# JonasGeiping/breaching

Hardware: NVIDIA B200
Metric: reconstruction iters/sec (ResNet-18 224x224, invertinggradients) (higher is better)
Workload: dtype tf32

## Files before the change

breaching_b200/csrc/engine.cu:

```cuda
#include <math.h>
#include <stdlib.h>
#include <string.h>

#include <limits>
#include <string>
#include <vector>

#include "../../include/breaching_b200.h"
#include "common.cuh"
#include "igemm.cuh"
#include "layers.cuh"
#include "tokens.cuh"
#include "objective.cuh"
#include "augment.cuh"

namespace bre {
void set_pdl(bool on);
static thread_local std::string g_last_error;
void set_error(const std::string& msg) { g_last_error = msg; }
static int g_pdl = -1;
bool use_pdl() {
  if (g_pdl < 0) {
    const char* e = getenv("BRE_PDL");
    g_pdl = e ? (atoi(e) != 0) : 1;
// ... 51 lines not shown
struct bre_engine {
  int device = 0;
  cudaStream_t stream = nullptr;
  std::vector<TensorBuf> t;
  std::vector<bre_op_desc> ops;
  std::vector<ParamInfo> params;
  std::vector<BnBuf> bn;
  std::vector<int*> pool_idx;
  int logits = -1;
  bre_attack_cfg cfg;
  std::vector<void*> allocs;

  long long P_pad = 0, max_param = 0, max_tensor = 0;
  float *W = nullptr, *g = nullptr, *G = nullptr, *V = nullptr, *stage = nullptr, *chunk_w = nullptr;
  float *Wt = nullptr, *Vt = nullptr;
  std::vector<float*> ms_Wt;
  bool tc_round_env = [] { const char* e = getenv("BRE_TC_ROUND"); return e ? atoi(e) != 0 : true; }();
  bool tc_round() const { return gemm_backend == 1 && tc_round_env; }
  float *p = nullptr, *loss_n = nullptr;
  long long* labels = nullptr;
  int seq_len = 0;
  std::vector<float*> tok_a, tok_b;
  float* soft_q = nullptr;
  float* soft_q_buf = nullptr;
  float* label_grad = nullptr;
  int n_labels = 0;
  int logits_valid = 0;
  int classes() const { return logits_valid > 0 ? logits_valid : td(logits).C; }
  bool joint = false;
  float *ell = nullptr, *ell_m = nullptr, *ell_v = nullptr, *ell_best = nullptr;
  long long n_ell = 0;
  long long nx = 0;
  int xN = 0, xC = 0, xH = 0, xW = 0;
  float *x = nullptr, *gradx = nullptr, *gradx_task = nullptr, *m = nullptr, *v = nullptr, *best = nullptr;
  float *history = nullptr, *lr_table = nullptr, *lo = nullptr, *hi = nullptr;
  int n_lr = 0, lr_cap = 0;
  Scalars* sc = nullptr;
  float* ws = nullptr;
  int ws_tiles = 0;
  int* gemm_counters = nullptr;
  float* red_partials = nullptr;
  int* red_counters = nullptr;
  double* dpartials = nullptr;
  int* dcounter = nullptr;
  DiLayer* di_layers_dev = nullptr;
  int n_di = 0;
  float* feat_measured = nullptr;
  long long feat_numel = 0;
  int feat_op = -1;
  cudaStream_t side = nullptr;
  std::vector<cudaEvent_t> ev_fork;
  cudaEvent_t ev_join = nullptr;
  bool overlap_wgrad = true;
  bool fuse_bnact = [] { const char* e = getenv("BRE_FUSE_BNACT"); return e ? atoi(e) != 0 : false; }();
  float* ws2 = nullptr;
  int* gemm_counters2 = nullptr;
  float* red_partials2 = nullptr;
  int* red_counters2 = nullptr;
  struct StepBufs {
    std::vector<float*> val, d;
    std::vector<int*> idx;
    std::vector<float*> bn_scale, bn_shift;
    float* p = nullptr; float* loss_n = nullptr; long long* labels = nullptr;
  };
  int ms_steps = 0;
  float ms_lr = 0.f;
  std::vector<float*> ms_W;
  std::vector<StepBufs> ms_bufs;
  std::vector<long long> ms_offset;
  float* ms_D = nullptr;
  float* gradx_step = nullptr;
  float* W0 = nullptr;
  struct BnPrep { int gamma_off, beta_off, C; const float* inv; const float* nrm; float* scale; float* shift; };
  std::vector<BnPrep*> ms_bnprep_dev;
  int n_bn_layers = 0;
  bool want_tangent_G = false;
  int stem_op = -1, stem_Kp = 0;
  float *xcol = nullptr, *dcol = nullptr, *Wcol = nullptr, *Vcol = nullptr, *Gcol = nullptr;
  bool stem_cols_env = [] { const char* e = getenv("BRE_STEM_COLS"); return e ? atoi(e) != 0 : true; }();
  bool use_stem_cols(size_t i) { return gemm_backend == 1 && stem_cols_env && (int)i == stem_op && !is_precise(i); }
  GemmArgs stem_geom(const bre_op_desc& op) const {
    GemmArgs a;
    memset(&a, 0, sizeof(a));
    const bre_tensor_desc& to = td(op.tout);
    a.g = ConvGeom{to.N, to.H, to.W, stem_Kp, to.H, to.W, to.C, 1, 1, 1, 0};
    a.x_sN = (long long)to.H * to.W * stem_Kp; a.x_sP = stem_Kp; a.x_sC = 1;
    a.nsrc = 1;
    a.ws = ws; a.counters = gemm_counters; a.ws_tiles = ws_tiles; a.splits = 0;
    return a;
  }
  int stem_unfold(const bre_op_desc& op) {
    const bre_tensor_desc &ti = td(op.tin), &to = td(op.tout);
    BRE_LAUNCH(launch_stem_im2col(t[0].val, xcol, ti.N, ti.C, ti.H, ti.W, to.H, to.W, op.R, op.S, op.stride, op.pad, stem_Kp, tc_round(), stream));
    return 0;
  }
  int stem_pad(const float* src, float* dst, const bre_op_desc& op, cudaStream_t st) {
    BRE_LAUNCH(launch_stem_pad_rows(src, dst, td(op.tout).C, op.R * op.S * td(op.tin).C, stem_Kp, false, tc_round(), st));
    return 0;
  }
  int stem_fold(const bre_op_desc& op, float* grad_out) {
    const bre_tensor_desc &ti = td(op.tin), &to = td(op.tout);
    BRE_LAUNCH(launch_stem_col2im(dcol, grad_out, ti.N, ti.C, ti.H, ti.W, to.H, to.W, op.R, op.S, op.stride, op.pad, stem_Kp, stream));
    return 0;
  }
  int precise_first = [] { const char* e = getenv("BRE_PRECISE_FIRST"); return e ? atoi(e) : 0; }();
  int precise_last = [] { const char* e = getenv("BRE_PRECISE_LAST"); return e ? atoi(e) : 0; }();
  mutable std::vector<char> precise_op;
// ... 116 lines not shown
    }
    if (stem_op >= 0 && stem_cols_env && !is_precise((size_t)stem_op)) rnd_d[ops[stem_op].tout] = 1;
  }
  bool round_val(int tensor) { if (rnd_val.size() != t.size()) compute_round_flags(); return tc_round() && rnd_val[tensor]; }
  bool round_d(int tensor) { if (rnd_d.size() != t.size()) compute_round_flags(); return tc_round() && rnd_d[tensor]; }

  GemmArgs conv_geom(const bre_op_desc& op) const {
    GemmArgs a;
    memset(&a, 0, sizeof(a));
    const bre_tensor_desc &ti = td(op.tin), &to = td(op.tout);
    ConvGeom& g = a.g;
    if (op.kind == BRE_OP_LINEAR) {
      g.N = ti.N; g.H = 1; g.W = 1; g.Ci = ti.C * ti.H * ti.W; g.Ho = 1; g.Wo = 1; g.Co = to.C;
      g.R = 1; g.S = 1; g.stride = 1; g.pad = 0;
      a.x_sN = g.Ci; a.x_sP = g.Ci; a.x_sC = 1;
    } else {
      g.N = ti.N; g.H = ti.H; g.W = ti.W; g.Ci = ti.C; g.Ho = to.H; g.Wo = to.W; g.Co = to.C;
      g.R = op.R; g.S = op.S; g.stride = op.stride; g.pad = op.pad;
      if (op.tin == 0) { a.x_sN = (long long)ti.C * ti.H * ti.W; a.x_sP = 1; a.x_sC = ti.H * ti.W; }
      else { a.x_sN = (long long)ti.H * ti.W * ti.C; a.x_sP = ti.C; a.x_sC = 1; }
    }
    a.nsrc = 1;
    a.ws = ws; a.counters = gemm_counters; a.ws_tiles = ws_tiles; a.splits = 0;
    a.force_fp32 = is_precise(op_index(op)) ? 1 : 0;
    return a;
  }
  int gemm(const GemmArgs& a) { return gemm_on(a, stream); }
  bool weight_prefetch = [] { const char* e = getenv("BRE_TC_WPREFETCH"); return e ? atoi(e) != 0 : true; }();
  bool v_settled = false;
  bool inside(const float* p, const float* base, long long n) const { return base != nullptr && p >= base && p < base + n; }
  unsigned static_weights(const GemmArgs& a) const {
    if (!weight_prefetch || ms_steps > 0 || a.mode == GEMM_WGRAD) return 0u;
    unsigned mask = 0;
    for (int s = 0; s < a.nsrc; ++s) {
      const float* p = a.wgt[s];
      const bool model = inside(p, W, P_pad) || inside(p, Wt, P_pad) || (Wcol != nullptr && p == Wcol);
      const bool direction = v_settled && (inside(p, V, P_pad) || inside(p, Vt, P_pad));
      if (model || direction) mask |= 1u << s;
    }
    return mask;
  }
  int gemm_on(const GemmArgs& a, cudaStream_t st) {
    if (linear_tall_supported(a)) return launch_linear_tall(a, st);
    if (linear_small_preferred(a)) return launch_linear_small(a, st);
    if (gemm_backend == 1 && !a.force_fp32 && igemm_tc_supported(a)) {
      GemmArgs b = a;
      b.wgt_static = static_weights(a);
      return launch_igemm_tc(b, st);
    }
    return launch_igemm_simt(a, st);
  }

  bool fuses_with_next(size_t i, const GemmArgs& a) const {
    if (!fuse_bnact || gemm_backend != 1 || i + 1 >= ops.size()) return false;
    const bre_op_desc& nx = ops[i + 1];
    return nx.kind == BRE_OP_BNACT && nx.tin == ops[i].tout && !nx.bn_train && igemm_tc_supported(a);
  }
  int consumers_of(int tensor) const {
    int n = 0;
    for (const bre_op_desc& o : ops) n += (o.tin == tensor) + (o.res == tensor);
    return n;
  }

  BnTrainArgs bn_train_args(const bre_op_desc& op) {
    const bre_tensor_desc& to = td(op.tout);
    const BnBuf& b = bn[op.bn_buffer];
    BnTrainArgs a;
    memset(&a, 0, sizeof(a));
    a.P = (long long)to.N * to.H * to.W; a.C = to.C; a.relu = op.relu != 0;
    a.in = t[op.tin].val; a.out = t[op.tout].val;
    a.inv = b.inv; a.nrm = b.nrm; a.scale = b.scale;
    a.v_gamma = Vp(op.gamma); a.v_beta = Vp(op.beta);
    a.sum_du = Gp(op.beta); a.sum_duxh = Gp(op.gamma);
    a.m1 = b.di_cm; a.m2 = b.di_cv; a.b1 = b.tb1; a.b2 = b.tb2;
    a.dout = t[op.tout].d; a.tdout = t[op.tout].td; a.xd = t[op.tin].tval;
    return a;
  }

  BnConsts bn_consts(const bre_op_desc& op) const {
    BnConsts c{nullptr, nullptr, nullptr, nullptr};
    if (op.has_bn) { const BnBuf& b = bn[op.bn_buffer]; c = BnConsts{b.scale, b.shift, b.inv, b.nrm}; }
    return c;
  }
  PoolGeom pool_geom(const bre_op_desc& op) const {
    const bre_tensor_desc &ti = td(op.tin), &to = td(op.tout);
    return PoolGeom{ti.N, ti.H, ti.W, ti.C, to.H, to.W, op.R, op.stride, op.pad};
  }
  bool need_task_grad() const { return cfg.task_regularization != 0.f; }
  float value_task_reg() const { return cfg.objective_excludes_task ? 0.f : cfg.task_regularization; }

  int sweep_forward() {
    for (size_t i = 0; i < ops.size(); ++i) {
      const bre_op_desc& op = ops[i];
      const bre_tensor_desc& to = td(op.tout);
      const long long Pout = (long long)to.N * to.H * to.W;
      switch (op.kind) {
        case BRE_OP_CONV:
        case BRE_OP_LINEAR: {
          GemmArgs a = conv_geom(op);
          a.mode = GEMM_FPROP;
          a.act[0] = t[op.tin].val; a.wgt[0] = Wg(op);
          if (use_stem_cols(i)) {
            BRE_TRY(stem_unfold(op));
            if (ms_steps > 0) BRE_TRY(stem_pad(Wp(op.w), Wcol, op, stream));
            a = stem_geom(op);
            a.mode = GEMM_FPROP;
            a.act[0] = xcol; a.wgt[0] = Wcol;
          }
          a.bias = op.b >= 0 ? Wp(op.b) : nullptr;
// ... 1390 lines not shown
```

breaching_b200/csrc/igemm.cuh:

```cuda
#pragma once
#include "common.cuh"

namespace bre {

enum GemmMode { GEMM_FPROP = 0, GEMM_DGRAD = 1, GEMM_WGRAD = 2 };

struct ConvGeom {
  int N, H, W, Ci;
  int Ho, Wo, Co;
  int R, S, stride, pad;
};

struct GemmEpilogue {
  int kind;
  int has_bn, relu;
  int round_out;
  float* out2;
  const float* res;
  const float* scale;
  const float* shift;
  const float* inv;
  const float* nrm;
  const float* v_gamma;
  const float* v_beta;
  const float* pre;
  const float* post;
};

struct GemmArgs {
  int mode;
  GemmEpilogue epi;
  ConvGeom g;
  int nsrc;
  const float* act[2];
  const float* wgt[2];
  long long x_sN;
  int x_sP, x_sC;
  float* out;
  const float* bias;
  int accumulate;
  float* ws;
  int* counters;
  int ws_tiles;
  int splits;
  int force_fp32;
  unsigned wgt_static;
};

constexpr int IG_BM = 64, IG_BN = 64, IG_BK = 16, IG_THREADS = 256;

int launch_igemm_simt(const GemmArgs& a, cudaStream_t stream);
bool linear_small_supported(const GemmArgs& a);
int launch_linear_small(const GemmArgs& a, cudaStream_t stream);
bool linear_small_preferred(const GemmArgs& a);
bool linear_tall_supported(const GemmArgs& a);
int launch_linear_tall(const GemmArgs& a, cudaStream_t stream);
int launch_igemm_tc(const GemmArgs& a, cudaStream_t stream);
bool igemm_tc_supported(const GemmArgs& a);

inline void gemm_dims(const GemmArgs& a, int& M, int& Nc, int& K) {
  const ConvGeom& g = a.g;
  if (a.mode == GEMM_FPROP) { M = g.N * g.Ho * g.Wo; Nc = g.Co; K = g.R * g.S * g.Ci; }
  else if (a.mode == GEMM_DGRAD) { M = g.N * g.H * g.W; Nc = g.Ci; K = g.R * g.S * g.Co; }
  else { M = g.Co; Nc = g.R * g.S * g.Ci; K = g.N * g.Ho * g.Wo; }
}

}
```

breaching_b200/csrc/igemm_tc.cu:

```cuda
#include <stdlib.h>
#include <string.h>

#include <array>
#include <map>
#include <mutex>
#include <type_traits>

#include <cuda.h>

#include "igemm.cuh"

namespace bre {

namespace {

constexpr int TC_BM = 128;
constexpr int TC_BK = 32;
constexpr int TC_STAGES = 4;
constexpr int TC_MAX_STAGES = 8;
constexpr int TC_THREADS = 128;
constexpr int TC_BLOCK = TC_THREADS + 32;

struct TcDims {
  int M, Nc, K;
// ... 106 lines not shown
constexpr int TC_MAXCLS = 4;
struct ClsPlan {
  int ncls, stride;
  int tile0[TC_MAXCLS + 1];
  int Hc[TC_MAXCLS], Wc[TC_MAXCLS], y0[TC_MAXCLS], x0[TC_MAXCLS];
  int Ty[TC_MAXCLS], Tx[TC_MAXCLS], Ly[TC_MAXCLS], Lx[TC_MAXCLS], ey[TC_MAXCLS], ex[TC_MAXCLS];
};
struct TcMapsCls {
  CUtensorMap act[2 * TC_MAXCLS];
  CUtensorMap wgt[2];
};

__device__ __forceinline__ void mbar_expect_tx(uint64_t* bar, uint32_t bytes) {
  asm volatile("mbarrier.arrive.expect_tx.shared::cta.b64 _, [%0], %1;" ::"r"(smem_u32(bar)), "r"(bytes) : "memory");
}
__device__ __forceinline__ void tma_im2col(uint32_t dst, const CUtensorMap* tm, uint64_t* bar, int c, int w, int h, int n, int ow, int oh) {
  asm volatile(
      "cp.async.bulk.tensor.4d.shared::cluster.global.im2col.mbarrier::complete_tx::bytes [%0], [%1, {%3, %4, %5, %6}], [%2], {%7, %8};"
      ::"r"(dst), "l"(reinterpret_cast<uint64_t>(tm)), "r"(smem_u32(bar)), "r"(c), "r"(w), "r"(h), "r"(n), "h"((uint16_t)ow), "h"((uint16_t)oh)
      : "memory");
}
__device__ __forceinline__ void tma_tile2d(uint32_t dst, const CUtensorMap* tm, uint64_t* bar, int c0, int c1) {
  asm volatile("cp.async.bulk.tensor.2d.shared::cluster.global.tile.mbarrier::complete_tx::bytes [%0], [%1, {%3, %4}], [%2];"
               ::"r"(dst), "l"(reinterpret_cast<uint64_t>(tm)), "r"(smem_u32(bar)), "r"(c0), "r"(c1) : "memory");
}
__device__ __forceinline__ void tma_tile3d(uint32_t dst, const CUtensorMap* tm, uint64_t* bar, int c0, int c1, int c2) {
  asm volatile("cp.async.bulk.tensor.3d.shared::cluster.global.tile.mbarrier::complete_tx::bytes [%0], [%1, {%3, %4, %5}], [%2];"
               ::"r"(dst), "l"(reinterpret_cast<uint64_t>(tm)), "r"(smem_u32(bar)), "r"(c0), "r"(c1), "r"(c2) : "memory");
}

template <int NV>
__device__ __forceinline__ void fused_bnact(const GemmEpilogue& e, long long row, int n, float (&v)[NV]) {
  const long long o = row + n;
#pragma unroll
  for (int j = 0; j < NV; ++j) {
    float u = v[j];
    if (e.kind == 1) {
      if (e.has_bn) u = fmaf(u, __ldg(e.scale + n + j), __ldg(e.shift + n + j));
      if (e.res != nullptr) u += e.res[o + j];
      u = e.relu ? fmaxf(u, 0.f) : u;
      v[j] = e.round_out ? tf32_rna(u) : u;
    } else {
      if (e.has_bn) {
        const float xhat = fmaf(e.pre[o + j], __ldg(e.inv + n + j), __ldg(e.nrm + n + j));
        u = fmaf(__ldg(e.scale + n + j), u, fmaf(__ldg(e.v_gamma + n + j), xhat, __ldg(e.v_beta + n + j)));
      }
      if (e.res != nullptr) u += e.res[o + j];
      if (e.relu && !(e.post[o + j] > 0.f)) u = 0.f;
      v[j] = e.round_out ? tf32_rna(u) : u;
    }
  }
}

#ifdef BRE_TC_TRACE
__device__ long long g_tc_trace[16];
#define TC_MARK(i, cond) do { if ((cond) && blockIdx.x == 0 && blockIdx.y == 0 && blockIdx.z == 0) g_tc_trace[i] = clock64(); } while (0)
#else
#define TC_MARK(i, cond) do { } while (0)
#endif

template <int MODE, int BN, bool TMA, bool CLS = false>
__global__ void __launch_bounds__(TC_BLOCK) igemm_tc_kernel(GemmArgs a, TcDims d, int proxy_fence,
                                                            const __grid_constant__ std::conditional_t<CLS, TcMapsCls, TcMaps> maps, ClsPlan plan) {
  static_assert(!CLS || (MODE == GEMM_DGRAD && TMA), "per-class gathers: strided dgrad with the TMA producer only");
  constexpr uint32_t A_BYTES = TC_BM * TC_BK * 4, B_BYTES = BN * TC_BK * 4;
  extern __shared__ __align__(1024) uint8_t smem[];
  uint8_t* sA = smem;
  const int nst = 1 << d.stage_shift, stage_mask = nst - 1;
  uint8_t* sB = smem + nst * A_BYTES;
  __shared__ __align__(8) uint64_t bar_full[TC_MAX_STAGES];
  __shared__ __align__(8) uint64_t bar_empty[TC_MAX_STAGES];
  __shared__ __align__(8) uint64_t bar_done;
  __shared__ uint32_t s_tmem;

  TC_MARK(0, threadIdx.x == 0);
  pdl_launch_dependents();
  const ConvGeom g = a.g;
  const int tid = threadIdx.x, warp = tid >> 5;
  const int n0 = blockIdx.y * BN, z = blockIdx.z;
  int m0 = blockIdx.x * TC_BM;
  int kb_begin = z * d.kblocks_per_split;
  int kb_end = min(d.total_kblocks, kb_begin + d.kblocks_per_split);
  const int HoWo = g.Ho * g.Wo, HW = g.H * g.W;
  int cls = 0, cHc = 0, cWc = 0, cTy = 0, cTx = 0, cls_kps = 0, Mrows = d.M;
  if (CLS) {
#pragma unroll
    for (int c = 1; c < TC_MAXCLS; ++c)
      if (c < plan.ncls && (int)blockIdx.x >= plan.tile0[c]) cls = c;
    m0 = ((int)blockIdx.x - plan.tile0[cls]) * TC_BM;
    cHc = plan.Hc[cls]; cWc = plan.Wc[cls]; cTy = plan.Ty[cls]; cTx = plan.Tx[cls];
    Mrows = g.N * cHc * cWc;
    cls_kps = cTy * cTx * (g.Co / TC_BK);
    const int total = cls_kps * a.nsrc, per = (total + (int)gridDim.z - 1) / (int)gridDim.z;
    kb_begin = z * per;
    kb_end = min(total, kb_begin + per);
  }

  if (tid == 0) {
#pragma unroll
    for (int s = 0; s < TC_MAX_STAGES; ++s) { mbar_init(&bar_full[s], TMA ? 1 : TC_THREADS); mbar_init(&bar_empty[s], 1); }
    mbar_init(&bar_done, 1);
    fence_barrier_init();
  }
  if (warp == 0) tmem_alloc(&s_tmem, BN);
  tc_fence_before();
  __syncthreads();
  tc_fence_after();
  const uint32_t tmem_d = s_tmem;
  TC_MARK(1, threadIdx.x == 0);

  constexpr uint32_t a_mn = (MODE == GEMM_WGRAD) ? 1u : 0u;
  constexpr uint32_t b_mn = (MODE == GEMM_FPROP) ? 0u : 1u;
  constexpr uint32_t idesc = (1u << 4) | (2u << 7) | (2u << 10) | (a_mn << 15) | (b_mn << 16) | ((uint32_t)(BN >> 3) << 17) |
                             ((uint32_t)(TC_BM >> 4) << 24);

  constexpr int A_VEC = TC_BM * TC_BK / 4 / TC_THREADS;
  constexpr int B_VEC = BN * TC_BK / 4 / TC_THREADS;
// ... 122 lines not shown
    } else if (MODE == GEMM_DGRAD) {
#pragma unroll
      for (int h = 0; h < BN / 32; ++h) tma_tile3d(pb + h * 4096, &maps.wgt[st.src], bar, n0 + 32 * h, st.rs, st.c0);
    } else {
      const uint32_t pa = smem_u32(sA) + stage * A_BYTES;
#pragma unroll
      for (int h = 0; h < TC_BM / 32; ++h) tma_tile2d(pa + h * 4096, &maps.wgt[st.src], bar, m0 + 32 * h, st.c0);
    }
  };
  auto issue_act_tma = [&](int stage, const KbState& st) {
    uint64_t* bar = &bar_full[stage];
    const uint32_t pa = smem_u32(sA) + stage * A_BYTES, pb = smem_u32(sB) + stage * B_BYTES;
    if (MODE == GEMM_FPROP) {
      tma_im2col(pa, &maps.act[st.src], bar, st.c0, base_w, base_h, base_n, st.s, st.r);
    } else if (MODE == GEMM_DGRAD) {
      if (CLS) tma_im2col(pa, &maps.act[2 * cls + st.src], bar, st.c0, base_w, base_h, base_n, cTx - 1 - st.s, cTy - 1 - st.r);
      else tma_im2col(pa, &maps.act[st.src], bar, st.c0, base_w, base_h, base_n, g.S - 1 - st.s, g.R - 1 - st.r);
    } else {
#pragma unroll
      for (int h = 0; h < BN / 32; ++h)
        tma_im2col(pb + h * 4096, &maps.act[st.src], bar, wg_c[h], st.q * g.stride - g.pad, st.p * g.stride - g.pad, st.img, wg_s[h], wg_r[h]);
    }
  };

  if (TMA && tid == 0 && (proxy_fence & 2)) {
    for (int sidx = 0; sidx < a.nsrc; ++sidx) {
      asm volatile("prefetch.tensormap [%0];" ::"l"(reinterpret_cast<uint64_t>(&maps.act[(CLS ? 2 * cls : 0) + sidx])) : "memory");
      asm volatile("prefetch.tensormap [%0];" ::"l"(reinterpret_cast<uint64_t>(&maps.wgt[sidx])) : "memory");
    }
  }
  const int nprod = (proxy_fence >> 2) & 7;
  const bool producer = TMA && (tid & 31) == 0 && warp < nprod && warp < nkb;
  KbState pst;
  memset(&pst, 0, sizeof(pst));
  uint32_t pre_wgt = 0;
  if (producer) {
    pst = kb_init(kb_begin + warp);
    if (MODE != GEMM_WGRAD && a.wgt_static != 0) {
      KbState st = pst;
      for (int i = warp; i < nkb && i < nst; i += nprod) {
        if ((a.wgt_static >> st.src) & 1) {
          mbar_expect_tx(&bar_full[i], A_BYTES + B_BYTES);
          issue_wgt_tma(i, st);
          pre_wgt |= 1u << i;
        }
        for (int u = 0; u < nprod; ++u) kb_advance(st);
      }
    }
  }

  pdl_wait();
  TC_MARK(2, threadIdx.x == 0);

  auto issue_block = [&](int stage) {
    const int src = it_src;
    const int kch = (MODE == GEMM_DGRAD) ? g.Co : g.Ci;
    const int kbase = (MODE == GEMM_WGRAD) ? it_c0 : it_rs * kch + it_c0;
    const float* __restrict__ act = a.act[src];
    const float* __restrict__ wgt = a.wgt[src];
    const uint32_t pa = smem_u32(sA + stage * A_BYTES), pb = smem_u32(sB + stage * B_BYTES);
    if (MODE == GEMM_FPROP) {
      const int r = it_rs / g.S, s = it_rs - r * g.S;
      const int tapoff = (r * g.W + s) * a.x_sP + it_c0;
#pragma unroll
      for (int j = 0; j < A_VEC; ++j) {
        const bool ok = (a_taps[j] >> it_rs) & 1ull;
        cp_async16(pa + off_k128(grow + 16 * j, gcol), ok ? act + (a_off[j] + tapoff) : act, ok ? 16u : 0u);
      }
      const float* q = wgt + (long long)(n0 + grow) * d.K + kbase + gcol * 4;
#pragma unroll
      for (int j = 0; j < B_VEC; ++j) cp_async16(pb + off_k128(grow + 16 * j, gcol), q + (long long)(16 * j) * d.K, 16u);
    } else if (MODE == GEMM_DGRAD) {
      const int rs = it_rs, k0 = it_c0;
      const int r = rs / g.S, s = rs - r * g.S;
      if (g.stride == 1) {
        const int tapoff = k0 - (r * g.Wo + s) * g.Co;
#pragma unroll
        for (int j = 0; j < A_VEC; ++j) {
          const bool ok = (a_taps[j] >> rs) & 1ull;
          cp_async16(pa + off_k128(grow + 16 * j, gcol), ok ? act + (a_off[j] + tapoff) : act, ok ? 16u : 0u);
        }
      } else {
        const bool st2 = g.stride == 2;
#pragma unroll
        for (int j = 0; j < A_VEC; ++j) {
          const bool ok = (a_taps[j] >> rs) & 1ull;
          const int dr = r - (a_yx[j] >> 16), ds = s - (a_yx[j] & 0xffff);
          const int tr = st2 ? dr >> 1 : dr / g.stride, ts = st2 ? ds >> 1 : ds / g.stride;
          cp_async16(pa + off_k128(grow + 16 * j, gcol), ok ? act + (a_off[j] + k0 - (tr * g.Wo + ts) * g.Co) : act, ok ? 16u : 0u);
        }
      }
      const int n4 = tid & 15, kk = tid >> 4;
#pragma unroll
      for (int j = 0; j < B_VEC; ++j) {
        const int k = kk + 8 * j;
        const float* gb = wgt + ((long long)(k0 + k) * (g.R * g.S) + rs) * g.Ci + n0 + n4 * 4;
        cp_async16(pb + off_mnmajor<BN>(4 * n4, k), gb, 16u);
      }
    } else {
      {
        const int m4 = tid & 31, kk = tid >> 5;
#pragma unroll
        for (int j = 0; j < A_VEC; ++j) {
          const int k = kk + 4 * j;
          const int pix = kbase + k;
          const bool kok = pix < d.K;
// ... 78 lines not shown
        const int stage = i & stage_mask;
        if (i >= nst) mbar_wait(&bar_empty[stage], (uint32_t)(((i >> d.stage_shift) - 1) & 1));
        issue_block(stage);
        cp_async_arrive(&bar_full[stage]);
      }
    }
    mbar_wait(&bar_done, 0);
    TC_MARK(6, tid == 0);
    tc_fence_after();
  }

  const int splits = gridDim.z;
  const int tile = blockIdx.y * gridDim.x + blockIdx.x;
  const uint32_t lane_base = tmem_d + ((uint32_t)(warp * 32) << 16);
  float v[32];
  const int m = m0 + tid;
  const bool row_ok = m < Mrows;
  const bool is_loader = warp < TC_THREADS / 32;
  auto out_row = [&](int mm, long long& row, int& cs) {
    if (CLS) {
      const int per = cHc * cWc;
      const int img = mm / per, rem = mm - img * per;
      const int iy = rem / cWc, ix = rem - iy * cWc;
      row = img * a.x_sN + (long long)((plan.y0[cls] + plan.stride * iy) * g.W + plan.x0[cls] + plan.stride * ix) * a.x_sP;
      cs = a.x_sC;
    } else if (MODE == GEMM_DGRAD) {
      const int img = mm / HW;
      row = img * a.x_sN + (long long)(mm - img * HW) * a.x_sP;
      cs = a.x_sC;
    } else {
      row = (long long)mm * d.Nc;
      cs = 1;
    }
  };
  if (!is_loader) {
  } else if (splits == 1) {
    long long row = 0;
    int cs = 1;
    if (row_ok) out_row(m, row, cs);
#pragma unroll
    for (int c = 0; c < BN; c += 32) {
      if (nkb > 0) tmem_ld32(lane_base + c, v);
      else {
#pragma unroll
        for (int j = 0; j < 32; ++j) v[j] = 0.f;
      }
      if (!row_ok) continue;
      const int n = n0 + c;
      if (MODE == GEMM_FPROP && a.bias != nullptr) {
#pragma unroll
        for (int j = 0; j < 32; ++j) v[j] += __ldg(a.bias + n + j);
      }
      float* op = a.out + row + (long long)n * cs;
      if (MODE == GEMM_FPROP && a.epi.kind != 0) {
        if (a.out != nullptr) {
#pragma unroll
          for (int j = 0; j < 32; j += 4) *reinterpret_cast<float4*>(op + j) = make_float4(v[j], v[j + 1], v[j + 2], v[j + 3]);
        }
        fused_bnact<32>(a.epi, row, n, v);
        float* op2 = a.epi.out2 + row + n;
#pragma unroll
        for (int j = 0; j < 32; j += 4) *reinterpret_cast<float4*>(op2 + j) = make_float4(v[j], v[j + 1], v[j + 2], v[j + 3]);
      } else if (cs == 1) {
#pragma unroll
        for (int j = 0; j < 32; j += 4) {
          float4 t = make_float4(v[j], v[j + 1], v[j + 2], v[j + 3]);
          if (a.accumulate) {
            const float4 o = *reinterpret_cast<const float4*>(op + j);
            t.x += o.x; t.y += o.y; t.z += o.z; t.w += o.w;
          }
          *reinterpret_cast<float4*>(op + j) = t;
        }
      } else {
#pragma unroll
        for (int j = 0; j < 32; ++j) {
          float* q = op + (long long)j * cs;
          *q = a.accumulate ? *q + v[j] : v[j];
        }
      }
    }
  } else {
    float* part = reinterpret_cast<float*>(sA);
#pragma unroll
    for (int c = 0; c < BN; c += 32) {
      if (nkb > 0) tmem_ld32(lane_base + c, v);
      else {
#pragma unroll
        for (int j = 0; j < 32; ++j) v[j] = 0.f;
      }
#pragma unroll
      for (int j = 0; j < 32; j += 4) {
        const int chunk = ((c + j) >> 2) ^ (tid & (BN / 4 - 1) & 15);
        *reinterpret_cast<float4*>(part + tid * BN + chunk * 4) = make_float4(v[j], v[j + 1], v[j + 2], v[j + 3]);
      }
    }
  }
  if (splits > 1) {
    TC_MARK(7, tid == 0);
    cluster_sync_all();
    TC_MARK(8, tid == 0);
    if (is_loader) {
      auto reduce_rows = [&](auto s_tag) {
        constexpr int S = decltype(s_tag)::value;
        constexpr int C4 = BN / 4, SLOTS = (TC_BM / S) * C4 / TC_THREADS > 0 ? (TC_BM / S) * C4 / TC_THREADS : 1;
        static_assert(BN >= 64 || S <= 8, "narrow tiles: at most 8 splits");
        const uint32_t part_s = smem_u32(sA);
        float4 t[SLOTS][S];
        int rr[SLOTS], cc[SLOTS];
#pragma unroll
        for (int sl = 0; sl < SLOTS; ++sl) {
          const int slot = tid + sl * TC_THREADS;
          rr[sl] = z * (TC_BM / S) + slot / C4;
          cc[sl] = slot % C4;
          const uint32_t local = part_s + (uint32_t)(rr[sl] * BN + ((cc[sl] ^ (rr[sl] & (BN / 4 - 1) & 15)) << 2)) * 4u;
#pragma unroll
          for (int q = 0; q < S; ++q) t[sl][q] = ld_dsmem4(local, (uint32_t)q);
        }
#pragma unroll
        for (int sl = 0; sl < SLOTS; ++sl) {
          const int r = rr[sl], c4 = cc[sl];
          if (m0 + r >= Mrows) continue;
          float4 acc4 = t[sl][0];
#pragma unroll
          for (int q = 1; q < S; ++q) { acc4.x += t[sl][q].x; acc4.y += t[sl][q].y; acc4.z += t[sl][q].z; acc4.w += t[sl][q].w; }
          const int n = n0 + c4 * 4;
          if (MODE == GEMM_FPROP && a.bias != nullptr) {
            acc4.x += __ldg(a.bias + n); acc4.y += __ldg(a.bias + n + 1); acc4.z += __ldg(a.bias + n + 2); acc4.w += __ldg(a.bias + n + 3);
          }
          long long row;
          int cs;
          out_row(m0 + r, row, cs);
          float* op = a.out + row + (long long)n * cs;
          if (MODE == GEMM_FPROP && a.epi.kind != 0) {
            if (a.out != nullptr) *reinterpret_cast<float4*>(op) = acc4;
            float vv[4] = {acc4.x, acc4.y, acc4.z, acc4.w};
            fused_bnact<4>(a.epi, row, n, vv);
            *reinterpret_cast<float4*>(a.epi.out2 + row + n) = make_float4(vv[0], vv[1], vv[2], vv[3]);
          } else if (cs == 1) {
            if (a.accumulate) {
              const float4 o = *reinterpret_cast<const float4*>(op);
              acc4.x += o.x; acc4.y += o.y; acc4.z += o.z; acc4.w += o.w;
            }
            *reinterpret_cast<float4*>(op) = acc4;
          } else {
            const float vv[4] = {acc4.x, acc4.y, acc4.z, acc4.w};
#pragma unroll
            for (int j = 0; j < 4; ++j) {
              float* qq = op + (long long)j * cs;
              *qq = a.accumulate ? *qq + vv[j] : vv[j];
            }
          }
        }
      };
      switch (splits) {
        case 2: reduce_rows(std::integral_constant<int, 2>{}); break;
        case 4: reduce_rows(std::integral_constant<int, 4>{}); break;
        case 8: reduce_rows(std::integral_constant<int, 8>{}); break;
        default:
          if constexpr (BN >= 64) reduce_rows(std::integral_constant<int, 16>{});
          break;
      }
    }
    TC_MARK(9, tid == 0);
    cluster_sync_all();
  }
  tc_fence_before();
  __syncthreads();
  if (warp == 0) tmem_dealloc(tmem_d, BN);
  TC_MARK(10, tid == 0);
}

inline bool aligned16(const void* p) { return (reinterpret_cast<uintptr_t>(p) & 15) == 0; }

typedef CUresult (*EncodeIm2colFn)(CUtensorMap*, CUtensorMapDataType, cuuint32_t, void*, const cuuint64_t*, const cuuint64_t*, const int*,
                                   const int*, cuuint32_t, cuuint32_t, const cuuint32_t*, CUtensorMapInterleave, CUtensorMapSwizzle,
                                   CUtensorMapL2promotion, CUtensorMapFloatOOBfill);
typedef CUresult (*EncodeTiledFn)(CUtensorMap*, CUtensorMapDataType, cuuint32_t, void*, const cuuint64_t*, const cuuint64_t*,
                                  const cuuint32_t*, const cuuint32_t*, CUtensorMapInterleave, CUtensorMapSwizzle,
                                  CUtensorMapL2promotion, CUtensorMapFloatOOBfill);

struct TmaApi {
  EncodeIm2colFn im2col = nullptr;
  EncodeTiledFn tiled = nullptr;
  int driver = 0;
  bool ok = false;
};
const TmaApi& tma_api() {
  static const TmaApi api = [] {
    TmaApi t;
    cudaDriverEntryPointQueryResult q;
// ... 118 lines not shown
}

bool cls_eligible(const GemmArgs& a) {
  static const int env = [] { const char* e = getenv("BRE_TC_STRIDED_TMA"); return e ? atoi(e) : 1; }();
  const ConvGeom& g = a.g;
  if (!env || a.mode != GEMM_DGRAD || g.stride != 2 || !tma_api().ok) return false;
  static const int tma_env = [] { const char* e = getenv("BRE_TC_TMA"); return e ? atoi(e) : 1; }();
  if (!tma_env || g.R > 16 || g.S > 16) return false;
  for (int ey = 0; ey < 2; ++ey)
    for (int horiz = 0; horiz < 2; ++horiz) {
      const AxisPlan p = horiz ? axis_plan(g.W, g.Wo, g.S, 2, g.pad, ey) : axis_plan(g.H, g.Ho, g.R, 2, g.pad, ey);
      if (p.any && p.T > 0 && (p.L < -128 || p.L > 127 || p.U < -128 || p.U > 127)) return false;
    }
  return true;
}

bool build_cls(const GemmArgs& a, ClsPlan* plan, TcMapsCls* maps) {
  const ConvGeom& g = a.g;
  memset(plan, 0, sizeof(*plan));
  plan->stride = g.stride;
  int tiles = 0, n = 0;
  for (int ey = 0; ey < g.stride; ++ey) {
    const AxisPlan py = axis_plan(g.H, g.Ho, g.R, g.stride, g.pad, ey);
    if (!py.any) continue;
    for (int ex = 0; ex < g.stride; ++ex) {
      const AxisPlan px = axis_plan(g.W, g.Wo, g.S, g.stride, g.pad, ex);
      if (!px.any) continue;
      if (n >= TC_MAXCLS) return false;
      const bool taps = py.T > 0 && px.T > 0;
      plan->Hc[n] = py.Hc; plan->Wc[n] = px.Hc; plan->y0[n] = py.y0; plan->x0[n] = px.y0;
      plan->Ty[n] = taps ? py.T : 0; plan->Tx[n] = taps ? px.T : 0;
      plan->Ly[n] = py.L; plan->Lx[n] = px.L; plan->ey[n] = ey; plan->ex[n] = ex;
      plan->tile0[n] = tiles;
      tiles += ceil_div((long long)g.N * py.Hc * px.Hc, TC_BM);
      for (int s = 0; s < a.nsrc && taps; ++s)
        if (!im2col_map(&maps->act[2 * n + s], a.act[s], g.N, g.Ho, g.Wo, g.Co, (long long)g.Ho * g.Wo * g.Co, g.Co, px.L, py.L, px.U, py.U, 1,
                        TC_BK, TC_BM, CU_TENSOR_MAP_SWIZZLE_128B))
          return false;
      if (!taps)
        for (int s = 0; s < a.nsrc; ++s) maps->act[2 * n + s] = maps->act[s];
      ++n;
    }
  }
  plan->ncls = n;
  plan->tile0[n] = tiles;
  for (int s = 0; s < a.nsrc; ++s) {
    const long long dims[3] = {g.Ci, (long long)g.R * g.S, g.Co}, strides[2] = {g.Ci, (long long)g.R * g.S * g.Ci};
    const int box[3] = {32, 1, TC_BK};
    if (!tiled_map(&maps->wgt[s], a.wgt[s], 3, dims, strides, box, CU_TENSOR_MAP_SWIZZLE_128B_ATOM_32B)) return false;
  }
  return n > 0;
}

template <int MODE, int BN, bool TMA, bool CLS = false>
int launch_tc(const GemmArgs& a, const TcDims& d0, const std::conditional_t<CLS, TcMapsCls, TcMaps>& maps, cudaStream_t stream,
              const ClsPlan* plan_in = nullptr) {
  TcDims d = d0;
  ClsPlan plan;
  memset(&plan, 0, sizeof(plan));
  if (CLS) plan = *plan_in;
  const int tm = CLS ? plan.tile0[plan.ncls] : ceil_div(d.M, TC_BM), tn = d.Nc / BN;
  if (CLS) {
    int kmax = 0;
    for (int c = 0; c < plan.ncls; ++c) kmax = kmax > plan.Ty[c] * plan.Tx[c] ? kmax : plan.Ty[c] * plan.Tx[c];
    d.total_kblocks = kmax * (a.g.Co / TC_BK) * a.nsrc;
    if (d.total_kblocks < 1) d.total_kblocks = 1;
  }
  const long long tiles = (long long)tm * tn;
  static const int max_splits_env = [] { const char* e = getenv("BRE_TC_MAX_SPLITS"); return e ? atoi(e) : 0; }();
  static const int target_ctas_env = [] { const char* e = getenv("BRE_TC_TARGET_CTAS"); return e ? atoi(e) : 0; }();
  const int target = target_ctas_env > 0 ? target_ctas_env : 144;
  constexpr int kMaxCluster = BN >= 64 ? 16 : 8;
  int splits = a.splits;
  if (splits <= 0) {
    splits = 1;
    while (splits < kMaxCluster && tiles * splits < target && d.total_kblocks / (splits * 2) >= 2) splits *= 2;
  }
  if (max_splits_env > 0 && splits > max_splits_env) splits = max_splits_env;
  int pow2 = 1;
  while (pow2 * 2 <= splits && pow2 < kMaxCluster) pow2 *= 2;
  splits = pow2;
  while (splits > 1 && splits > d.total_kblocks) splits /= 2;
  d.kblocks_per_split = ceil_div(d.total_kblocks, splits);
  if (tn > 65535) { set_error("igemm_tc: grid too large"); return -1; }
  static const int stages_env = [] { const char* e = getenv("BRE_TC_STAGES"); return e ? atoi(e) : 0; }();
  static const int shortk_env = [] { const char* e = getenv("BRE_TC_SHORTK_STAGES"); return e ? atoi(e) : 2; }();
  const bool shortk = shortk_env == 2 && d.kblocks_per_split <= 6 && tm == 1 && tiles * splits > 2LL * kNumSMs;
  const int stages = (stages_env == 8 || stages_env == 2) ? stages_env : (shortk ? 2 : TC_STAGES);
  d.stage_shift = stages == 8 ? 3 : (stages == 2 ? 1 : 2);
  const size_t smem = (size_t)stages * (TC_BM + BN) * TC_BK * 4;
  const size_t smem_max = (size_t)TC_MAX_STAGES * (TC_BM + BN) * TC_BK * 4;
  static bool attr_done = false;
  if (!attr_done) {
    BRE_CUDA_CHECK(cudaFuncSetAttribute(igemm_tc_kernel<MODE, BN, TMA, CLS>, cudaFuncAttributeMaxDynamicSharedMemorySize, (int)smem_max));
    BRE_CUDA_CHECK(cudaFuncSetAttribute(igemm_tc_kernel<MODE, BN, TMA, CLS>, cudaFuncAttributeNonPortableClusterSizeAllowed, 1));
    attr_done = true;
  }
  static const int proxy_fence_env = [] {
    const char* e = getenv("BRE_TC_PROXY_FENCE");
    const char* pf = getenv("BRE_TC_PREFETCH");
    const char* np = getenv("BRE_TC_PRODUCERS");
    int nprod = np ? atoi(np) : 2;
    if (nprod < 1 || nprod > 4) nprod = 2;
    return (e && atoi(e) ? 1 : 0) | ((pf ? atoi(pf) : 1) ? 2 : 0) | (nprod << 2);
  }();
  {
    cudaError_t lerr = launch_kernel(igemm_tc_kernel<MODE, BN, TMA, CLS>, dim3(tm, tn, splits), dim3(TC_BLOCK), smem, stream, splits, a, d,
                                     proxy_fence_env, maps, plan);
    if (lerr != cudaSuccess) { set_error(std::string("igemm_tc launch failed: ") + cudaGetErrorString(lerr)); return -2; }
  }
  BRE_CHECK_LAUNCH();
  return 0;
}

}

static bool narrow_tiles_ok(const GemmArgs& a) {
  static const int env = [] { const char* e = getenv("BRE_TC_NARROW"); return e ? atoi(e) : 1; }();
  if (!env || !tma_eligible(a)) return false;
  if (a.mode == GEMM_DGRAD && a.g.stride != 1) return false;
  if (a.mode == GEMM_WGRAD && (a.g.Ci % 32 != 0)) return false;
  return true;
}

bool igemm_tc_supported(const GemmArgs& a) {
  const ConvGeom& g = a.g;
  int M, Nc, K;
  gemm_dims(a, M, Nc, K);
  for (int s = 0; s < a.nsrc; ++s)
    if (!aligned16(a.act[s]) || !aligned16(a.wgt[s])) return false;
  if (!aligned16(a.out) || (a.splits == 0 && a.ws == nullptr)) return false;
  const bool x_nhwc = a.x_sC == 1 && a.x_sP % 4 == 0 && a.x_sN % 4 == 0;
  if (Nc % 64 != 0 && !(Nc % 32 == 0 && narrow_tiles_ok(a))) return false;
  switch (a.mode) {
    case GEMM_FPROP: return x_nhwc && g.Ci % TC_BK == 0 && g.R * g.S <= 64;
    case GEMM_DGRAD: return x_nhwc && g.Co % TC_BK == 0 && g.R * g.S <= 64;
    case GEMM_WGRAD: return x_nhwc && g.Co % 4 == 0 && g.Ci % 4 == 0 && g.R * g.S <= 64;
    default: return false;
  }
}

int launch_igemm_tc(const GemmArgs& a, cudaStream_t stream) {
  if (!igemm_tc_supported(a)) { set_error("igemm_tc: unsupported shape"); return -4; }
  TcDims d;
  gemm_dims(a, d.M, d.Nc, d.K);
  d.kblocks_per_src = ceil_div(d.K, TC_BK);
  d.total_kblocks = d.kblocks_per_src * a.nsrc;
  d.kblocks_per_split = d.total_kblocks;
  TcMaps maps;
  memset(&maps, 0, sizeof(maps));
  if (cls_eligible(a)) {
    ClsPlan plan;
    TcMapsCls cmaps;
    memset(&cmaps, 0, sizeof(cmaps));
    if (build_cls(a, &plan, &cmaps)) return launch_tc<GEMM_DGRAD, 64, true, true>(a, d, cmaps, stream, &plan);
  }
  if (d.Nc % 64 != 0) {
    if (!build_maps(a, 32, &maps)) { set_error("igemm_tc: tensor-map encoding failed for a narrow-tile shape"); return -4; }
    if (a.mode == GEMM_FPROP) return launch_tc<GEMM_FPROP, 32, true>(a, d, maps, stream);
    if (a.mode == GEMM_DGRAD) return launch_tc<GEMM_DGRAD, 32, true>(a, d, maps, stream);
    return launch_tc<GEMM_WGRAD, 32, true>(a, d, maps, stream);
  }
  const bool tma = tma_eligible(a) && build_maps(a, 64, &maps);
  if (a.mode == GEMM_FPROP) return tma ? launch_tc<GEMM_FPROP, 64, true>(a, d, maps, stream) : launch_tc<GEMM_FPROP, 64, false>(a, d, maps, stream);
  if (a.mode == GEMM_DGRAD) return tma ? launch_tc<GEMM_DGRAD, 64, true>(a, d, maps, stream) : launch_tc<GEMM_DGRAD, 64, false>(a, d, maps, stream);
  return tma ? launch_tc<GEMM_WGRAD, 64, true>(a, d, maps, stream) : launch_tc<GEMM_WGRAD, 64, false>(a, d, maps, stream);
}

}

#ifdef BRE_TC_TRACE
extern "C" int bre_debug_tc_trace(long long* out16) {
  return cudaMemcpyFromSymbol(out16, bre::g_tc_trace, sizeof(long long) * 16) == cudaSuccess ? 0 : -1;
}
#endif
```

Baseline: 941.2.

## Enable fused BN/residual/ReLU epilogue in TMA fprop GEMM with prefetched operands

Turns on GEMM+BN-activation fusion by default and restricts it to TMA fprop launches with 64-wide tiles and at least four K-splits. For those launches a dedicated kernel variant prefetches the residual, pre/post activation and per-channel BN vectors before the main loop, so the split-K epilogue applies BN, residual and ReLU without extra dependent loads. The aim is to remove separate elementwise bnact kernel launches and their memory round trips. The cost is higher register pressure and a new kernel instantiation, and the fusion is turned off in multi-step mode.

```diff
diff --git a/breaching_b200/csrc/engine.cu b/breaching_b200/csrc/engine.cu
--- a/breaching_b200/csrc/engine.cu
+++ b/breaching_b200/csrc/engine.cu
@@ -127,7 +127,7 @@
   std::vector<cudaEvent_t> ev_fork;
   cudaEvent_t ev_join = nullptr;
   bool overlap_wgrad = true;
-  bool fuse_bnact = [] { const char* e = getenv("BRE_FUSE_BNACT"); return e ? atoi(e) != 0 : false; }();
+  bool fuse_bnact = [] { const char* e = getenv("BRE_FUSE_BNACT"); return e ? atoi(e) != 0 : true; }();
   float* ws2 = nullptr;
   int* gemm_counters2 = nullptr;
   float* red_partials2 = nullptr;
@@ -350,9 +350,10 @@
   }
 
   bool fuses_with_next(size_t i, const GemmArgs& a) const {
-    if (!fuse_bnact || gemm_backend != 1 || i + 1 >= ops.size()) return false;
+    if (!fuse_bnact || gemm_backend != 1 || ms_steps > 0 || i + 1 >= ops.size()) return false;
     const bre_op_desc& nx = ops[i + 1];
-    return nx.kind == BRE_OP_BNACT && nx.tin == ops[i].tout && !nx.bn_train && igemm_tc_supported(a);
+    return nx.kind == BRE_OP_BNACT && nx.tin == ops[i].tout && !nx.bn_train && !a.force_fp32 && !linear_tall_supported(a) &&
+           !linear_small_preferred(a) && igemm_tc_fuses_epilogue(a);
   }
   int consumers_of(int tensor) const {
     int n = 0;
diff --git a/breaching_b200/csrc/igemm.cuh b/breaching_b200/csrc/igemm.cuh
--- a/breaching_b200/csrc/igemm.cuh
+++ b/breaching_b200/csrc/igemm.cuh
@@ -57,6 +57,7 @@
 int launch_linear_tall(const GemmArgs& a, cudaStream_t stream);
 int launch_igemm_tc(const GemmArgs& a, cudaStream_t stream);
 bool igemm_tc_supported(const GemmArgs& a);
+bool igemm_tc_fuses_epilogue(const GemmArgs& a);
 
 inline void gemm_dims(const GemmArgs& a, int& M, int& Nc, int& K) {
   const ConvGeom& g = a.g;
diff --git a/breaching_b200/csrc/igemm_tc.cu b/breaching_b200/csrc/igemm_tc.cu
--- a/breaching_b200/csrc/igemm_tc.cu
+++ b/breaching_b200/csrc/igemm_tc.cu
@@ -182,6 +182,32 @@
   }
 }
 
+__device__ __forceinline__ float4 fused_bnact4(const GemmEpilogue& e, float4 acc, float4 res, float4 pre, float4 post, const float4 (&c)[5]) {
+  float u[4] = {acc.x, acc.y, acc.z, acc.w};
+  const float r[4] = {res.x, res.y, res.z, res.w}, z[4] = {pre.x, pre.y, pre.z, pre.w}, o[4] = {post.x, post.y, post.z, post.w};
+  const float c0[4] = {c[0].x, c[0].y, c[0].z, c[0].w}, c1[4] = {c[1].x, c[1].y, c[1].z, c[1].w};
+  const float c2[4] = {c[2].x, c[2].y, c[2].z, c[2].w}, c3[4] = {c[3].x, c[3].y, c[3].z, c[3].w};
+  const float c4[4] = {c[4].x, c[4].y, c[4].z, c[4].w};
+#pragma unroll
+  for (int j = 0; j < 4; ++j) {
+    if (e.kind == 1) {
+      if (e.has_bn) u[j] = fmaf(u[j], c0[j], c1[j]);
+      if (e.res != nullptr) u[j] += r[j];
+      u[j] = e.relu ? fmaxf(u[j], 0.f) : u[j];
+    } else {
+      if (e.has_bn) {
+        const float xhat = fmaf(z[j], c1[j], c2[j]);
+        u[j] = fmaf(c0[j], u[j], fmaf(c3[j], xhat, c4[j]));
+      }
+      if (e.res != nullptr) u[j] += r[j];
+      if (e.relu && !(o[j] > 0.f)) u[j] = 0.f;
+    }
+    u[j] = e.round_out ? tf32_rna(u[j]) : u[j];
+  }
+  return make_float4(u[0], u[1], u[2], u[3]);
+}
+__device__ __forceinline__ float4 ldg_f4(const float* p, long long i4) { return __ldg(reinterpret_cast<const float4*>(p) + i4); }
+
 #ifdef BRE_TC_TRACE
 __device__ long long g_tc_trace[16];
 #define TC_MARK(i, cond) do { if ((cond) && blockIdx.x == 0 && blockIdx.y == 0 && blockIdx.z == 0) g_tc_trace[i] = clock64(); } while (0)
@@ -189,10 +215,11 @@
 #define TC_MARK(i, cond) do { } while (0)
 #endif
 
-template <int MODE, int BN, bool TMA, bool CLS = false>
+template <int MODE, int BN, bool TMA, bool CLS = false, bool EPI = false>
 __global__ void __launch_bounds__(TC_BLOCK) igemm_tc_kernel(GemmArgs a, TcDims d, int proxy_fence,
                                                             const __grid_constant__ std::conditional_t<CLS, TcMapsCls, TcMaps> maps, ClsPlan plan) {
   static_assert(!CLS || (MODE == GEMM_DGRAD && TMA), "per-class gathers: strided dgrad with the TMA producer only");
+  static_assert(!EPI || (MODE == GEMM_FPROP && TMA && !CLS && BN == 64), "fused epilogue: TMA fprop with 128 x 64 tiles only");
   constexpr uint32_t A_BYTES = TC_BM * TC_BK * 4, B_BYTES = BN * TC_BK * 4;
   extern __shared__ __align__(1024) uint8_t smem[];
   uint8_t* sA = smem;
@@ -421,6 +448,40 @@
   pdl_wait();
   TC_MARK(2, threadIdx.x == 0);
 
+  constexpr int EPI_PF = 4;
+  float4 e_res[EPI_PF], e_pre[EPI_PF], e_post[EPI_PF], e_c[5];
+  if constexpr (EPI) {
+    const float4 zero4 = make_float4(0.f, 0.f, 0.f, 0.f);
+#pragma unroll
+    for (int sl = 0; sl < EPI_PF; ++sl) e_res[sl] = e_pre[sl] = e_post[sl] = zero4;
+#pragma unroll
+    for (int q = 0; q < 5; ++q) e_c[q] = zero4;
+    const int S = gridDim.z;
+    if (S >= 4 && warp < TC_THREADS / 32) {
+      const GemmEpilogue& e = a.epi;
+      constexpr int C4 = BN / 4;
+      const int nsl = (TC_BM / S) * C4 / TC_THREADS, n = n0 + (tid % C4) * 4;
+#pragma unroll
+      for (int sl = 0; sl < EPI_PF; ++sl) {
+        const int mm = m0 + z * (TC_BM / S) + (tid + sl * TC_THREADS) / C4;
+        if (sl >= nsl || mm >= Mrows) continue;
+        const long long o4 = ((long long)mm * d.Nc + n) >> 2;
+        if (e.res != nullptr) e_res[sl] = ldg_f4(e.res, o4);
+        if (e.kind == 2 && e.has_bn) e_pre[sl] = ldg_f4(e.pre, o4);
+        if (e.kind == 2 && e.relu) e_post[sl] = ldg_f4(e.post, o4);
+      }
+      if (e.has_bn) {
+        e_c[0] = ldg_f4(e.scale, n >> 2);
+        if (e.kind == 1) {
+          e_c[1] = ldg_f4(e.shift, n >> 2);
+        } else {
+          e_c[1] = ldg_f4(e.inv, n >> 2); e_c[2] = ldg_f4(e.nrm, n >> 2);
+          e_c[3] = ldg_f4(e.v_gamma, n >> 2); e_c[4] = ldg_f4(e.v_beta, n >> 2);
+        }
+      }
+    }
+  }
+
   auto issue_block = [&](int stage) {
     const int src = it_src;
     const int kch = (MODE == GEMM_DGRAD) ? g.Co : g.Ci;
@@ -605,7 +666,7 @@
         for (int j = 0; j < 32; ++j) v[j] += __ldg(a.bias + n + j);
       }
       float* op = a.out + row + (long long)n * cs;
-      if (MODE == GEMM_FPROP && a.epi.kind != 0) {
+      if (EPI) {
         if (a.out != nullptr) {
 #pragma unroll
           for (int j = 0; j < 32; j += 4) *reinterpret_cast<float4*>(op + j) = make_float4(v[j], v[j + 1], v[j + 2], v[j + 3]);
@@ -684,11 +745,18 @@
           int cs;
           out_row(m0 + r, row, cs);
           float* op = a.out + row + (long long)n * cs;
-          if (MODE == GEMM_FPROP && a.epi.kind != 0) {
+          if constexpr (EPI) {
             if (a.out != nullptr) *reinterpret_cast<float4*>(op) = acc4;
-            float vv[4] = {acc4.x, acc4.y, acc4.z, acc4.w};
-            fused_bnact<4>(a.epi, row, n, vv);
-            *reinterpret_cast<float4*>(a.epi.out2 + row + n) = make_float4(vv[0], vv[1], vv[2], vv[3]);
+            float4 y;
+            if constexpr (S >= 4) {
+              static_assert(SLOTS <= EPI_PF, "prefetched slots");
+              y = fused_bnact4(a.epi, acc4, e_res[sl], e_pre[sl], e_post[sl], e_c);
+            } else {
+              float vv[4] = {acc4.x, acc4.y, acc4.z, acc4.w};
+              fused_bnact<4>(a.epi, row, n, vv);
+              y = make_float4(vv[0], vv[1], vv[2], vv[3]);
+            }
+            *reinterpret_cast<float4*>(a.epi.out2 + row + n) = y;
           } else if (cs == 1) {
             if (a.accumulate) {
               const float4 o = *reinterpret_cast<const float4*>(op);
@@ -913,7 +981,25 @@
   return n > 0;
 }
 
-template <int MODE, int BN, bool TMA, bool CLS = false>
+int tc_splits(long long tiles, int total_kblocks, int requested, int BN) {
+  static const int max_splits_env = [] { const char* e = getenv("BRE_TC_MAX_SPLITS"); return e ? atoi(e) : 0; }();
+  static const int target_ctas_env = [] { const char* e = getenv("BRE_TC_TARGET_CTAS"); return e ? atoi(e) : 0; }();
+  const int target = target_ctas_env > 0 ? target_ctas_env : 144;
+  const int max_cluster = BN >= 64 ? 16 : 8;
+  int splits = requested;
+  if (splits <= 0) {
+    splits = 1;
+    while (splits < max_cluster && tiles * splits < target && total_kblocks / (splits * 2) >= 2) splits *= 2;
+  }
+  if (max_splits_env > 0 && splits > max_splits_env) splits = max_splits_env;
+  int pow2 = 1;
+  while (pow2 * 2 <= splits && pow2 < max_cluster) pow2 *= 2;
+  splits = pow2;
+  while (splits > 1 && splits > total_kblocks) splits /= 2;
+  return splits;
+}
+
+template <int MODE, int BN, bool TMA, bool CLS = false, bool EPI = false>
 int launch_tc(const GemmArgs& a, const TcDims& d0, const std::conditional_t<CLS, TcMapsCls, TcMaps>& maps, cudaStream_t stream,
               const ClsPlan* plan_in = nullptr) {
   TcDims d = d0;
@@ -928,20 +1014,7 @@
     if (d.total_kblocks < 1) d.total_kblocks = 1;
   }
   const long long tiles = (long long)tm * tn;
-  static const int max_splits_env = [] { const char* e = getenv("BRE_TC_MAX_SPLITS"); return e ? atoi(e) : 0; }();
-  static const int target_ctas_env = [] { const char* e = getenv("BRE_TC_TARGET_CTAS"); return e ? atoi(e) : 0; }();
-  const int target = target_ctas_env > 0 ? target_ctas_env : 144;
-  constexpr int kMaxCluster = BN >= 64 ? 16 : 8;
-  int splits = a.splits;
-  if (splits <= 0) {
-    splits = 1;
-    while (splits < kMaxCluster && tiles * splits < target && d.total_kblocks / (splits * 2) >= 2) splits *= 2;
-  }
-  if (max_splits_env > 0 && splits > max_splits_env) splits = max_splits_env;
-  int pow2 = 1;
-  while (pow2 * 2 <= splits && pow2 < kMaxCluster) pow2 *= 2;
-  splits = pow2;
-  while (splits > 1 && splits > d.total_kblocks) splits /= 2;
+  const int splits = tc_splits(tiles, d.total_kblocks, a.splits, BN);
   d.kblocks_per_split = ceil_div(d.total_kblocks, splits);
   if (tn > 65535) { set_error("igemm_tc: grid too large"); return -1; }
   static const int stages_env = [] { const char* e = getenv("BRE_TC_STAGES"); return e ? atoi(e) : 0; }();
@@ -953,8 +1026,8 @@
   const size_t smem_max = (size_t)TC_MAX_STAGES * (TC_BM + BN) * TC_BK * 4;
   static bool attr_done = false;
   if (!attr_done) {
-    BRE_CUDA_CHECK(cudaFuncSetAttribute(igemm_tc_kernel<MODE, BN, TMA, CLS>, cudaFuncAttributeMaxDynamicSharedMemorySize, (int)smem_max));
-    BRE_CUDA_CHECK(cudaFuncSetAttribute(igemm_tc_kernel<MODE, BN, TMA, CLS>, cudaFuncAttributeNonPortableClusterSizeAllowed, 1));
+    BRE_CUDA_CHECK(cudaFuncSetAttribute(igemm_tc_kernel<MODE, BN, TMA, CLS, EPI>, cudaFuncAttributeMaxDynamicSharedMemorySize, (int)smem_max));
+    BRE_CUDA_CHECK(cudaFuncSetAttribute(igemm_tc_kernel<MODE, BN, TMA, CLS, EPI>, cudaFuncAttributeNonPortableClusterSizeAllowed, 1));
     attr_done = true;
   }
   static const int proxy_fence_env = [] {
@@ -966,7 +1039,7 @@
     return (e && atoi(e) ? 1 : 0) | ((pf ? atoi(pf) : 1) ? 2 : 0) | (nprod << 2);
   }();
   {
-    cudaError_t lerr = launch_kernel(igemm_tc_kernel<MODE, BN, TMA, CLS>, dim3(tm, tn, splits), dim3(TC_BLOCK), smem, stream, splits, a, d,
+    cudaError_t lerr = launch_kernel(igemm_tc_kernel<MODE, BN, TMA, CLS, EPI>, dim3(tm, tn, splits), dim3(TC_BLOCK), smem, stream, splits, a, d,
                                      proxy_fence_env, maps, plan);
     if (lerr != cudaSuccess) { set_error(std::string("igemm_tc launch failed: ") + cudaGetErrorString(lerr)); return -2; }
   }
@@ -1001,6 +1074,14 @@
   }
 }
 
+bool igemm_tc_fuses_epilogue(const GemmArgs& a) {
+  if (a.mode != GEMM_FPROP || !igemm_tc_supported(a) || !tma_eligible(a)) return false;
+  int M, Nc, K;
+  gemm_dims(a, M, Nc, K);
+  if (Nc % 64 != 0) return false;
+  return tc_splits((long long)ceil_div(M, TC_BM) * (Nc / 64), ceil_div(K, TC_BK) * a.nsrc, a.splits, 64) >= 4;
+}
+
 int launch_igemm_tc(const GemmArgs& a, cudaStream_t stream) {
   if (!igemm_tc_supported(a)) { set_error("igemm_tc: unsupported shape"); return -4; }
   TcDims d;
@@ -1010,6 +1091,13 @@
   d.kblocks_per_split = d.total_kblocks;
   TcMaps maps;
   memset(&maps, 0, sizeof(maps));
+  if (a.epi.kind != 0) {
+    if (a.mode != GEMM_FPROP || d.Nc % 64 != 0 || !tma_eligible(a) || !build_maps(a, 64, &maps)) {
+      set_error("igemm_tc: a fused epilogue needs an fprop with 64-wide tiles on the TMA producer");
+      return -4;
+    }
+    return launch_tc<GEMM_FPROP, 64, true, false, true>(a, d, maps, stream);
+  }
   if (cls_eligible(a)) {
     ClsPlan plan;
     TcMapsCls cmaps;
diff --git a/profiles/critical_path.py b/profiles/critical_path.py
--- /dev/null
+++ b/profiles/critical_path.py
@@ -0,0 +1,107 @@
+import argparse
+import collections
+import json
+import os
+import re
+import sys
+import tempfile
+
+ROOT = os.path.dirname(os.path.dirname(os.path.abspath(__file__)))
+sys.path.insert(0, ROOT)
+import torch
+
+import bench
+
+ELEMENTWISE = re.compile(r"^bnact_(fwd|bwd|tan_fwd|tan_bwd)")
+
+
+def short(name):
+    name = name.replace("(anonymous namespace)::", "").replace("void ", "")
+    return re.sub(r"\b\w+::", "", re.sub(r"\(.*$", "", name))
+
+
+def main():
+    ap = argparse.ArgumentParser()
+    ap.add_argument("--config", type=int, default=2)
+    ap.add_argument("--iters", type=int, default=20)
+    ap.add_argument("--warmup", type=int, default=20)
+    ap.add_argument("--graph", type=int, default=1)
+    ap.add_argument("--fuse-bnact", type=int, default=None, help="set the engine option fuse_bnact (default: leave it)")
+    ap.add_argument("--out", default=os.path.join(tempfile.gettempdir(), "critical_path"))
+    args = ap.parse_args()
+    os.makedirs(args.out, exist_ok=True)
+
+    dev = torch.device("cuda:0")
+    torch.cuda.set_device(dev)
+    case = bench.build_case(args.config)
+    runner = bench.EngineRunner(args.config, case, dev, "tc", 0)
+    eng = runner.eng
+    eng.set_option("use_graph", args.graph)
+    if args.fuse_bnact is not None:
+        eng.set_option("fuse_bnact", args.fuse_bnact)
+    runner.warm(args.warmup)
+    launches = eng.launches_per_iteration()
+
+    from torch.profiler import ProfilerActivity, profile
+
+    with profile(activities=[ProfilerActivity.CPU, ProfilerActivity.CUDA]) as prof:
+        eng.run(args.iters)
+        eng.sync()
+    trace = os.path.join(args.out, f"trace_c{args.config}.pt.trace.json")
+    prof.export_chrome_trace(trace)
+    with open(trace) as f:
+        events = json.load(f)["traceEvents"]
+    kernels = [e for e in events if e.get("cat") == "kernel" and e.get("ph") == "X"]
+    by_stream = collections.Counter(e["args"]["stream"] for e in kernels)
+    main_stream = by_stream.most_common(1)[0][0]
+    chain = sorted((e for e in kernels if e["args"]["stream"] == main_stream), key=lambda e: e["ts"])
+    n_it = args.iters
+
+    rows = collections.defaultdict(lambda: [0, 0.0, 0.0])
+    overlap = 0
+    prev_end = None
+    per_launch = []
+    for e in chain:
+        end = e["ts"] + e["dur"]
+        if prev_end is None:
+            prev_end = e["ts"]
+        if e["ts"] < prev_end:
+            overlap += 1
+        r = rows[short(e["name"])]
+        r[0] += 1
+        r[1] += max(0.0, end - prev_end)
+        r[2] += e["dur"]
+        per_launch.append((short(e["name"]), e["dur"], max(0.0, end - prev_end)))
+        prev_end = max(prev_end, end)
+    span = (chain[-1]["ts"] + chain[-1]["dur"] - chain[0]["ts"]) / n_it
+    total_chain = sum(r[1] for r in rows.values()) / n_it
+    ew = [(k, r) for k, r in rows.items() if ELEMENTWISE.match(k)]
+    ew_chain = sum(r[1] for _, r in ew) / n_it
+    ew_launch = sum(r[0] for _, r in ew) / n_it
+
+    lines = [
+        f"# config {args.config}, {'graph replay' if args.graph else 'eager launches'}, fuse_bnact="
+        f"{'default' if args.fuse_bnact is None else args.fuse_bnact}, {n_it} traced iterations, "
+        f"{torch.cuda.get_device_name(dev)}",
+        f"# engine launches/iteration {launches}; kernels traced {len(kernels)} ({len(kernels) / n_it:.1f}/iteration); "
+        f"streams {dict(by_stream)}; main stream {main_stream}: {len(chain) / n_it:.1f} launches/iteration, "
+        f"{overlap} overlapping starts",
+        f"# main-stream span {span:.1f} us/iteration, summed chain time {total_chain:.1f} us/iteration",
+        f"# BN/residual/ReLU element-wise kernels: {ew_launch:.1f} launches/iteration, chain time {ew_chain:.1f} us/iteration "
+        f"({100 * ew_chain / max(span, 1e-9):.1f} % of the span)",
+        "#   chain us/it   own us/it   launches/it   chain us/launch   kernel",
+    ]
+    for k, r in sorted(rows.items(), key=lambda kv: -kv[1][1]):
+        lines.append(f"    {r[1] / n_it:9.1f}   {r[2] / n_it:9.1f}   {r[0] / n_it:9.1f}   {r[1] / max(r[0], 1):9.2f}   {k}")
+    text = "\n".join(lines) + "\n"
+    print(text)
+    with open(os.path.join(args.out, f"critical_path_c{args.config}.txt"), "w") as f:
+        f.write(text)
+    with open(os.path.join(args.out, f"critical_path_c{args.config}_launches.csv"), "w") as f:
+        f.write("kernel,own_us,chain_us\n")
+        f.writelines(f'"{k}",{d:.3f},{c:.3f}\n' for k, d, c in per_launch)
+    eng.close()
+
+
+if __name__ == "__main__":
+    main()
```

After: 975.6, median of 6. 3.7% higher.
